# social-ai-uoft/sorrel

Hardware: AMD Instinct MI355X
Metric: agent-steps/sec (higher is better)
Workload: dtype u8 grid, f32 obs

## Files before the change

sorrel_amd/csrc/common.h:

```cpp
#pragma once


constexpr int kBlock = 256;
constexpr int kWave = 64;
constexpr int kMaxPass = 2;

struct DevTables {
    uint32_t thr_lo[SGW_MAX_TYPES];
    uint32_t delta[4][SGW_MAX_TYPES];
    double value[SGW_MAX_TYPES];
    uint8_t spawn_choice[SGW_MAX_TYPES][SGW_MAX_CHOICES];
    uint8_t spawn_count[SGW_MAX_TYPES];
    uint8_t agent_type[SGW_MAX_AGENTS];
    uint8_t dense_choice[SGW_MAX_CHOICES];
    uint8_t layer_fill[8];
    uint8_t layer_border[8];
    uint8_t pad_[8];
    uint8_t rule[SGW_MAX_TYPES];
    int8_t rule_layer[SGW_MAX_TYPES];
    uint8_t rule_become[SGW_MAX_TYPES];
    uint8_t pad2_[SGW_MAX_TYPES];
    uint32_t rule_mask[SGW_MAX_TYPES];
    uint32_t delta3[SGW_MAX_TYPES];
    double appearance[SGW_MAX_TYPES][SGW_MAX_CHANNELS];
// ... 13 lines not shown
    int64_t row[SGW_MAX_AGENTS];
    int64_t cap[SGW_MAX_AGENTS];
    int64_t step[SGW_MAX_AGENTS];
    void* states[SGW_MAX_AGENTS];
    float* rewards[SGW_MAX_AGENTS];
    int64_t* actions[SGW_MAX_AGENTS];
    float* dones[SGW_MAX_AGENTS];
    int64_t row_elems[SGW_MAX_AGENTS];
    uint64_t eps_thr[SGW_MAX_AGENTS];
};

struct RowPtrs {
    void* p[SGW_MAX_AGENTS];
    int64_t stride;
    const void* agent_action;
    int action_kind;
    float* reward_row;
    int64_t* action_row;
    const TurnState* ts;
    const TurnState* ets;
    int dual;
    int rows_mode2;
};

struct Params {
    int H, W, L, A, r, V, VV, C, T, nact, zA;
    int cells;
    int64_t env_stride;
    int cells_pad;
    int env_lds;
    int tab_bytes;
    uint32_t default_type, fill_type;
    uint32_t spawn_mask, thr_full_mask, pass_mask;
    uint32_t become_mask;
    uint32_t agent_mask;
    uint32_t dy_pack, dx_pack;
    uint32_t fill_delta[4];
    uint32_t fill_delta3;
    uint32_t fill_delta16[2];
    uint32_t spawn_pat;
    uint32_t spawn_thr;
    uint32_t spawn_full;
    uint32_t spawn_n;
    uint32_t choice_lo, choice_hi;
    uint32_t seed_lo, seed_hi;
    uint32_t first_env;
    int64_t E;
    uint32_t epoch, turn, flags;
    int a0, a1;
    int do_move;
    int obs_post;
    int obs_u8;
    int agent_rule;
    uint32_t tag_it, tag_notit;
    double tag_reward;
    uint8_t* agent_state;
    uint8_t* agent_dir;
    int has_become;
    uint32_t quiet0, quiet1;
    uint32_t kind_pack;
    int beam_radius;
    uint32_t clean_beam, zap_beam, beam_block_mask;
    int total_factor;
    uint8_t* state_at_pov;
    uint64_t dense_thr;
    int dense_count;
    uint8_t* grid;
    uint8_t* pos;
    uint8_t* actions;
    float* obs;
    float* rewards;
    double* total;
    const DevTables* tab;
    const uint8_t* tmpl;
    int* status;
    int obs_stage;
    int stage_agents;
    int obs_next;
    int obs_A, obs_a0;
    int64_t obs_ag;
    int big_pitch;
    int big_stage;
    int big_stage_off;
    uint32_t* walk_ctr;
    int walk_word;
    int walk_static;
    int single_spawner;
    int rows_mode;
    int rows_by_agent;
    int onehot;
    int tail_kind, tail_len;
    const float* tail_table;
    const TurnState* ts;
    uint32_t nturns;
    int64_t ts_obs, ts_act, ts_rew;
    uint32_t extras;
    uint32_t drawn_mask;
    uint8_t* target_types;
};
constexpr uint32_t kExtraDrawn = 1u, kExtraTargets = 2u;
#ifdef SGW_JIT
constexpr bool kExtrasDefault = false;
#else
constexpr bool kExtrasDefault = true;
#endif
constexpr bool extras_default_tables(const int tc) { return kExtrasDefault && tc == 0; }
template <bool XTRAS>
__device__ __forceinline__ uint32_t extras_of(const Params& p) {
    if constexpr (XTRAS) return p.extras;
    else return 0u;
}

struct U4 {
    uint32_t x, y, z, w;
};

__device__ __forceinline__ uint32_t xor3(uint32_t a, uint32_t b, uint32_t k) {
    uint32_t d;
    asm("v_bitop3_b32 %0, %1, %2, %3 bitop3:0x96" : "=v"(d) : "v"(a), "v"(b), "s"(k));
    return d;
}

template <bool OWN_KEYS = true>
__device__ __forceinline__ U4 philox4x32_10(uint32_t c0, uint32_t c1, uint32_t c2, uint32_t c3,
                                            uint32_t k0, uint32_t k1) {
#ifndef SGW_DIAG_SHARED_KEYS
    if constexpr (OWN_KEYS) asm volatile("" : "+s"(k0), "+s"(k1));
#endif
#pragma unroll
    for (int r = 0; r < 10; ++r) {
        const uint64_t p0 = (uint64_t)0xD2511F53u * c0;
        const uint64_t p1 = (uint64_t)0xCD9E8D57u * c2;
        const uint32_t n0 = xor3((uint32_t)(p1 >> 32), c1, k0);
        const uint32_t n2 = xor3((uint32_t)(p0 >> 32), c3, k1);
        c1 = (uint32_t)p1;
        c3 = (uint32_t)p0;
        c0 = n0;
        c2 = n2;
        k0 += 0x9E3779B9u;
        k1 += 0xBB67AE85u;
    }
    return U4{c0, c1, c2, c3};
}

__device__ __forceinline__ uint32_t opaque(uint32_t v) {
    asm volatile("" : "+v"(v));
    return v;
}

__device__ __forceinline__ uint32_t word_of(const U4& v, int i) {
    return i == 0 ? v.x : i == 1 ? v.y : i == 2 ? v.z : v.w;
}

__device__ __forceinline__ uint32_t value_draw(const Params& p, const uint32_t cell, const uint32_t turn, const uint32_t env_id, const uint32_t ep4) {
    const U4 w = philox4x32_10(cell >> 2, turn, env_id, ep4 | SGW_STREAM_VALUE, p.seed_lo, p.seed_hi);
    return word_of(w, (int)(cell & 3u));
}
__device__ __forceinline__ double drawn_value(const DevTables* gtab, const uint32_t t, const uint32_t u, const double otherwise) {
    return (uint64_t)u < gtab->alt_thr[t & 31u] ? gtab->value_alt[t & 31u] : otherwise;
}

__device__ __forceinline__ float obs_finish(double acc, int post) {
    if (post == SGW_OBS_POST_CLIP255_DIV255) acc = fmin(fmax(acc, 0.0), 255.0) / 255.0;
    return (float)acc;
}

template <int WPE>
__device__ __forceinline__ void gsync() {
    if constexpr (WPE == 1) {
        __builtin_amdgcn_fence(__ATOMIC_ACQ_REL, "wavefront");
        __builtin_amdgcn_wave_barrier();
    } else {
        __syncthreads();
    }
}

template <int G>
__device__ __forceinline__ void load_grid(const Params& p, const uint8_t* __restrict__ src,
                                          uint8_t* lds, int gtid) {
    if ((p.env_stride & 15) == 0 && p.env_stride >= p.cells_pad) {
        const uint4* s = reinterpret_cast<const uint4*>(src);
        uint4* d = reinterpret_cast<uint4*>(lds);
        const int nu = p.cells_pad >> 4;
        for (int i = gtid; i < nu; i += G) {
            uint4 v = s[i];
            if (i == nu - 1 && (p.cells & 15)) {
                const int tail = p.cells & 15;
                uint32_t w[4] = {v.x, v.y, v.z, v.w};
#pragma unroll
                for (int q = 0; q < 4; ++q) {
                    const int keep = tail - 4 * q;
                    if (keep <= 0) w[q] = 0xFFFFFFFFu;
                    else if (keep < 4) w[q] |= 0xFFFFFFFFu << (8 * keep);
                }
                v = make_uint4(w[0], w[1], w[2], w[3]);
            }
            d[i] = v;
        }
    } else if ((p.cells & 3) == 0 && (p.env_stride & 3) == 0) {
        const uint32_t* s = reinterpret_cast<const uint32_t*>(src);
        uint32_t* d = reinterpret_cast<uint32_t*>(lds);
        for (int i = gtid; i < (p.cells >> 2); i += G) d[i] = s[i];
    } else {
        for (int i = gtid; i < p.cells_pad; i += G) lds[i] = i < p.cells ? src[i] : (uint8_t)0xFF;
    }
}

template <int G>
__device__ __forceinline__ void store_grid(const Params& p, uint8_t* __restrict__ dst,
                                           const uint8_t* lds, int gtid) {
    if ((p.env_stride & 15) == 0 && p.env_stride >= p.cells_pad) {
        uint4* d = reinterpret_cast<uint4*>(dst);
        const uint4* s = reinterpret_cast<const uint4*>(lds);
        for (int i = gtid; i < (p.cells_pad >> 4); i += G) d[i] = s[i];
    } else if ((p.cells & 3) == 0 && (p.env_stride & 3) == 0) {
        uint32_t* d = reinterpret_cast<uint32_t*>(dst);
        const uint32_t* s = reinterpret_cast<const uint32_t*>(lds);
        for (int i = gtid; i < (p.cells >> 2); i += G) d[i] = s[i];
    } else {
        for (int i = gtid; i < p.cells; i += G) dst[i] = lds[i];
    }
}


template <int G>
__device__ __forceinline__ void sweep_single(const Params& p, uint8_t* lds_grid, uint32_t env_id, int gtid, uint32_t turn, const uint32_t ep4,
                                             uint32_t* through = nullptr,
                                             const int d0 = 0) {
    uint32_t* g32 = reinterpret_cast<uint32_t*>(lds_grid);
    const int ndw = (p.cells + 3) >> 2;
    for (int d = d0 + gtid; d < ndw; d += G) {
        const uint32_t dv = g32[d], pat = p.spawn_pat & 0xFFu;
        const bool m0 = (dv & 0xFFu) == pat, m1 = ((dv >> 8) & 0xFFu) == pat, m2 = ((dv >> 16) & 0xFFu) == pat, m3 = (dv >> 24) == pat;
        if (!(m0 | m1 | m2 | m3)) continue;
        const U4 w = philox4x32_10((uint32_t)d, turn, env_id, ep4 | SGW_STREAM_SPAWN, p.seed_lo, p.seed_hi);
        const bool f = p.spawn_full != 0;
        uint32_t hits = 0;
        hits |= (m0 && (f || w.x < p.spawn_thr)) ? 1u : 0u;
        hits |= (m1 && (f || w.y < p.spawn_thr)) ? 2u : 0u;
        hits |= (m2 && (f || w.z < p.spawn_thr)) ? 4u : 0u;
        hits |= (m3 && (f || w.w < p.spawn_thr)) ? 8u : 0u;
        if (hits == 0) continue;
        const U4 k = philox4x32_10((uint32_t)d, turn, env_id, ep4 | SGW_STREAM_SPAWN_KIND, p.seed_lo, p.seed_hi);
#pragma unroll
        for (int b = 0; b < 4; ++b)
            if ((hits >> b) & 1u) {
                const uint32_t pick = __umulhi(word_of(k, b), p.spawn_n);
                lds_grid[4 * d + b] = (uint8_t)(((pick < 4 ? p.choice_lo : p.choice_hi) >> (8 * (pick & 3u))) & 0xFFu);
            }
        if (through) through[d] = g32[d];
    }
}

template <int G>
__device__ __forceinline__ void sweep(const Params& p, const DevTables* tab, uint8_t* lds_grid,
                                      uint32_t env_id, int gtid, uint32_t turn, const uint32_t ep4) {
    uint32_t* g32 = reinterpret_cast<uint32_t*>(lds_grid);
    const int ndw = (p.cells + 3) >> 2;
    const uint32_t c3 = ep4 | SGW_STREAM_SPAWN;
    for (int d = gtid; d < ndw; d += G) {
        uint32_t v = g32[d];
        uint32_t m = 0;
#pragma unroll
        for (int b = 0; b < 4; ++b) {
            const uint32_t t = (v >> (8 * b)) & 0xFFu;
            const uint32_t is = (t < SGW_MAX_TYPES) ? ((p.spawn_mask >> t) & 1u) : 0u;
            m |= is << b;
        }
        if (m == 0) continue;
        const U4 w = philox4x32_10((uint32_t)d, turn, env_id, c3, p.seed_lo, p.seed_hi);
        uint32_t hits = 0;
#pragma unroll
        for (int b = 0; b < 4; ++b) {
            if ((m >> b) & 1u) {
                const uint32_t t = (v >> (8 * b)) & 31u;
                const bool hit = ((p.thr_full_mask >> t) & 1u) || (word_of(w, b) < tab->thr_lo[t]);
                hits |= (hit ? 1u : 0u) << b;
            }
        }
        if (hits == 0) continue;
        const U4 k = philox4x32_10((uint32_t)d, turn, env_id, ep4 | SGW_STREAM_SPAWN_KIND,
                                   p.seed_lo, p.seed_hi);
#pragma unroll
        for (int b = 0; b < 4; ++b) {
            if ((hits >> b) & 1u) {
                const uint32_t t = (v >> (8 * b)) & 31u;
                const uint32_t n = tab->spawn_count[t];
                const uint32_t pick = (uint32_t)(((uint64_t)word_of(k, b) * n) >> 32);
                const uint32_t nt = tab->spawn_choice[t][pick];
                v = (v & ~(0xFFu << (8 * b))) | (nt << (8 * b));
            }
        }
        g32[d] = v;
    }
}

template <int WPE, int G, typename Tab>
__device__ __forceinline__ void sweep_ordered(const Params& p, const Tab* rt, uint8_t* lg, const uint32_t env_id, const int gtid,
                                              const uint32_t turn, const uint32_t ep4, const int L, const int HW) {
    const uint32_t* lg32 = reinterpret_cast<const uint32_t*>(lg);
    for (int z = 0; z < L; ++z) {
        const int lo = z * HW, hi = lo + HW;
        for (int d = (lo >> 2) + gtid; d < ((hi + 3) >> 2); d += G) {
            const uint32_t word = lg32[d];
            if (word == p.quiet0 || word == p.quiet1) continue;
            uint32_t tj[4];
// ... 54 lines not shown
```

sorrel_amd/csrc/step_fast.h:

```cpp
#pragma once

constexpr int kMaxUnits = 4;
constexpr int kMaxUnitsRules = 8;
constexpr int kMaxUnitsPlain = 11;
constexpr size_t kLdsPerCu = 160 * 1024;
constexpr size_t kCacheResidentGrid = (size_t)288 << 20;

#define OBS_STORE(ptr, val) (*(ptr) = (val))


template <bool OWN_KEYS>
__device__ __forceinline__ uint32_t sweep_hits(const uint4& u, const uint32_t unit, const Params& p, const uint32_t env_id, const uint32_t turn, const uint32_t ep4) {
    uint32_t hits = 0;
    const uint32_t pat = p.spawn_pat & 0xFFu;
#pragma unroll
    for (int k = 0; k < 4; ++k) {
        const uint32_t dv = k == 0 ? u.x : k == 1 ? u.y : k == 2 ? u.z : u.w;
        const bool m0 = (dv & 0xFFu) == pat, m1 = ((dv >> 8) & 0xFFu) == pat, m2 = ((dv >> 16) & 0xFFu) == pat, m3 = (dv >> 24) == pat;
        if (m0 | m1 | m2 | m3) {
            const U4 w = philox4x32_10<OWN_KEYS>(opaque(unit * 4 + k), turn, env_id, ep4 | SGW_STREAM_SPAWN, p.seed_lo, p.seed_hi);
            const bool f = p.spawn_full != 0;
            uint32_t hb = 0;
            hb |= (m0 && (f || w.x < p.spawn_thr)) ? 1u : 0u;
            hb |= (m1 && (f || w.y < p.spawn_thr)) ? 2u : 0u;
            hb |= (m2 && (f || w.z < p.spawn_thr)) ? 4u : 0u;
            hb |= (m3 && (f || w.w < p.spawn_thr)) ? 8u : 0u;
            hits |= hb << (4 * k);
        }
    }
    return hits;
}

template <bool OWN_KEYS>
__device__ __forceinline__ void sweep_apply(uint32_t hits, const uint32_t unit, uint8_t* lg, const Params& p,
                                            const uint32_t env_id, const uint32_t turn, const uint32_t ep4) {
    while (hits) {
        const uint32_t cell = (uint32_t)__ffs(hits) - 1u;
        hits &= hits - 1u;
        const uint32_t off = unit * 16u + cell;
        const U4 kw = philox4x32_10<OWN_KEYS>(opaque(off >> 2), turn, env_id, ep4 | SGW_STREAM_SPAWN_KIND, p.seed_lo, p.seed_hi);
        const uint32_t pick = __umulhi(word_of(kw, off & 3u), p.spawn_n);
        lg[off] = (uint8_t)(((pick < 4 ? p.choice_lo : p.choice_hi) >> (8 * (pick & 3u))) & 0xFFu);
    }
}

#ifdef SGW_STAMPS
constexpr int kStampEnvs = 65536;
__device__ unsigned long long g_stamps[kStampEnvs * 8];
#define STAMP(i)                                                                                             \
    do {                                                                                                     \
        __builtin_amdgcn_sched_barrier(0);                                                                   \
        unsigned long long t_;                                                                               \
        asm volatile("s_memrealtime %0\n\ts_waitcnt lgkmcnt(0)" : "=s"(t_)::"memory");                             \
        __builtin_amdgcn_sched_barrier(0);                                                                   \
        if (lane == 0 && (i) > 0 && env < kStampEnvs) g_stamps[env * 8 + (i)-1] = t_ - tprev_;                \
        tprev_ = t_;                                                                                         \
    } while (0)
#else
#define STAMP(i)
#endif

#ifndef SGW_FAST_RULES_PLAIN_WAVES
#define SGW_FAST_RULES_PLAIN_WAVES 6
#endif
#ifndef SGW_FAST_MULTI_WAVES
#define SGW_FAST_MULTI_WAVES 6
#endif
template <int TL, int TC, int TR, int TH, int TW, bool TAIL = false>
__device__ __forceinline__ void fast_rows_emit(const Params& p, const RowPtrs* rp, uint8_t* smem, const int sub, const int lane) {
    typedef float vfloat4 __attribute__((ext_vector_type(4)));
    typedef float vfloat2 __attribute__((ext_vector_type(2)));
    constexpr int kN = TC * (2 * TR + 1) * (2 * TR + 1);
    const int ob_off = p.tab_bytes + ((TL * TH * TW + 15) & ~15);
    const int64_t env_first = (int64_t)blockIdx.x * 4;
    const int live = (int)(p.E - env_first < 4 ? p.E - env_first : 4);
    __syncthreads();
    auto emit_run = [&](float* dst, const int a, const int k0, const int n) {
        const uintptr_t ad = reinterpret_cast<uintptr_t>(dst);
        const int T = n * kN;
        auto src16 = [&](const int t) -> uint32_t {
            const int k = t / (kN / 2), j2 = t - k * (kN / 2);
            return *reinterpret_cast<const uint16_t*>(smem + (k0 + k) * p.env_lds + ob_off + a * kN + 2 * j2);
        };
        if ((kN & 1) == 0 && (ad & 15u) == 0) {
            const int q = T >> 2;
            const int mis = (int)((ad >> 4) & 7u);
            for (int i = lane - mis; i < q; i += 64) {
                if (i < 0) continue;
                const uint32_t lo = src16(2 * i), hi = src16(2 * i + 1);
                vfloat4 v;
                v.x = (float)(lo & 0xFFu);
                v.y = (float)(lo >> 8);
                v.z = (float)(hi & 0xFFu);
                v.w = (float)(hi >> 8);
                __builtin_nontemporal_store(v, reinterpret_cast<vfloat4*>(dst) + i);
            }
            if ((T & 3) && lane == 0) {
                const uint32_t b = src16(2 * q);
                vfloat2 v;
                v.x = (float)(b & 0xFFu);
                v.y = (float)(b >> 8);
                __builtin_nontemporal_store(v, reinterpret_cast<vfloat2*>(dst) + 2 * q);
            }
        } else if ((kN & 1) == 0 && (ad & 7u) == 0) {
            const int mis = (int)((ad >> 3) & 15u);
            for (int i = lane - mis; i < (T >> 1); i += 64) {
                if (i < 0) continue;
                const uint32_t b = src16(i);
                vfloat2 v;
                v.x = (float)(b & 0xFFu);
                v.y = (float)(b >> 8);
                __builtin_nontemporal_store(v, reinterpret_cast<vfloat2*>(dst) + i);
            }
        } else {
            for (int i = lane; i < T; i += 64) {
                const int k = i / kN, j = i - k * kN;
                __builtin_nontemporal_store((float)smem[(k0 + k) * p.env_lds + ob_off + a * kN + j], dst + i);
            }
        }
    };
    for (int a = sub; a < p.A; a += 4) {
        float* base = static_cast<float*>(rp->p[a]) + env_first * rp->stride;
        if (rp->stride == kN) emit_run(base, a, 0, live);
        else for (int k = 0; k < live; ++k) emit_run(base + k * rp->stride, a, k, 1);
        if (rp->dual && rp->ts->cap[a] > 0 && rp->ts->states[a]) {
            const int64_t re = rp->ts->row_elems[a];
            float* ring = static_cast<float*>(rp->ts->states[a]) + (rp->ts->row[a] * p.E + env_first) * re;
            if (re == kN) emit_run(ring, a, 0, live);
            else for (int k = 0; k < live; ++k) emit_run(ring + k * re, a, k, 1);
        }
        if constexpr (TAIL) if (p.tail_kind != SGW_TAIL_NONE && rp->stride >= kN + p.tail_len) {
            for (int k = 0; k < live; ++k) {
                float* t = base + k * rp->stride + kN;
                const int64_t ea = (env_first + k) * p.A + a;
                if (p.tail_kind == SGW_TAIL_AGENT_IS_IT) {
                    if (lane == 0) t[0] = (p.agent_state && p.agent_state[ea] == p.tag_it) ? 1.f : 0.f;
                } else {
                    const uint32_t yx = reinterpret_cast<const uint16_t*>(p.pos)[ea];
                    const float* src = p.tail_table + ((int64_t)(yx & 0xFFu) * TW + (yx >> 8)) * p.tail_len;
                    for (int j = lane; j < p.tail_len; j += 64) t[j] = src[j];
                }
            }
        }
    }
}

template <bool ONEHOT, int TL, int TC, int TR, int TH, int TW, bool TAG, bool RULES, bool STAGE, bool MULTI, bool P3, bool I16, bool ROWS, bool ROWX = false, bool TAIL = false, bool XTRAS = kExtrasDefault>
__device__ __forceinline__ void step_fast_body(const Params p, [[maybe_unused]] const RowPtrs* rp) {
    static_assert(!ROWS || (ONEHOT && TL && TC && TH && TW && !RULES && !STAGE && !MULTI && !P3 && !I16), "ROWS: plain or Tag movers, one-hot, compile-time shape");
    static_assert(!ROWX || (ONEHOT && STAGE && !MULTI && !I16 && !ROWS), "ROWX: a chunk-staging single-turn instance");
    extern __shared__ __attribute__((aligned(16))) uint8_t smem[];
    const int tid = threadIdx.x;
    const int lane = tid & 63;
    const int sub = __builtin_amdgcn_readfirstlane(tid >> 6);
    const int64_t env = (int64_t)blockIdx.x * 4 + sub;
    if (env >= p.E) {
        if constexpr (ROWS)
            if (p.obs_stage > 0 && p.a0 == 0 && p.a1 == p.A && !(p.flags & SGW_STEP_NO_OBS))
                fast_rows_emit<TL, TC, TR, TH, TW, TAIL>(p, rp, smem, sub, lane);
        return;
    }
#ifdef SGW_STAMPS
    unsigned long long tprev_ = 0;
    STAMP(0);
    if (lane == 0 && env < kStampEnvs) {
        g_stamps[env * 8 + 6] = tprev_;
        g_stamps[env * 8 + 7] = (unsigned long long)__builtin_amdgcn_s_getreg(63492) | ((unsigned long long)__builtin_amdgcn_s_getreg(63508) << 32);
    }
#endif

    const int L = TL ? TL : p.L;
    const int C = TC ? TC : p.C;
    const int r = TR ? TR : p.r;
    const int V = 2 * r + 1, VV = V * V;
    const int H = TH ? TH : p.H, W = TW ? TW : p.W, HW = H * W;
    constexpr bool kStatic = TL && TH && TW;
    constexpr bool kOwnKeys = !kStatic;
    const int cells = kStatic ? TL * TH * TW : p.cells;
    const int nunits = (cells + 15) >> 4;
    constexpr int NU = kStatic ? ((TL * TH * TW + 15) / 16 + 63) / 64 : kMaxUnits;
    constexpr int kFullRounds = kStatic ? ((TL * TH * TW + 15) / 16) / 64 : 0;
    constexpr int kTailUnits = kStatic ? ((TL * TH * TW + 15) / 16) % 64 : 0;
    constexpr bool kTailDword = kStatic && !RULES && kTailUnits > 0 && kTailUnits <= 48;
    const int zoff = p.zA * HW;
    static_assert(!I16 || (ONEHOT && !P3 && !RULES && !(TL && TH && TW)), "I16: a byte-staging instance with run-time map");
    constexpr int NW = P3 ? 1 : I16 ? 2 : (TC ? (TC + 3) / 4 : 4);
    constexpr int CMAX = P3 ? (TC ? TC : 10) : I16 ? (TC ? TC : 4) : 4 * NW;

    uint8_t* wl = smem + sub * p.env_lds;
    const DevTables* gtab = p.tab;
    const uint32_t env_id = p.first_env + (uint32_t)env;
    uint32_t turn0 = p.turn, ep4 = p.epoch << 4;
    if (p.ts) { turn0 = p.ts->turn + 1u; ep4 = p.ts->epoch << 4; }

    uint4 u[NU];
    {
        const uint4* src = reinterpret_cast<const uint4*>(p.grid + env * p.env_stride);
#pragma unroll
        for (int k = 0; k < NU; ++k)
            if (lane + 64 * k < nunits) u[k] = src[lane + 64 * k];
    }
    const bool mine = lane >= p.a0 && lane < p.a1 && lane < p.A;
    const bool rnd = (p.flags & SGW_STEP_RANDOM_ACTIONS) != 0;
    uint32_t yx = 0, act = 0;
    if (lane < p.A) yx = reinterpret_cast<const uint16_t*>(p.pos)[env * p.A + lane];
    if ((yx & 0xFFu) >= (uint32_t)H || (yx >> 8) >= (uint32_t)W) {
        yx = 0;
        atomicOr(p.status, SGW_STATUS_BAD_POS);
    }
    if (mine && p.do_move && !rnd) act = p.actions[env * p.A + lane];
    const double vtab = gtab->value[lane & 31];
    uint32_t atype = gtab->agent_type[lane];
    if (p.agent_state && lane < p.A) atype = p.agent_state[env * p.A + lane];
    uint32_t pov_type = atype;
    if constexpr (ONEHOT) {
        uint32_t* wd = reinterpret_cast<uint32_t*>(wl);
        if constexpr (I16) {
            wd[lane] = reinterpret_cast<const uint32_t*>(gtab->delta16)[lane];
            float* l = reinterpret_cast<float*>(smem + 4 * p.env_lds);
#pragma unroll
            for (int j = 0; j < 4; ++j) l[lane + 64 * j] = gtab->post_lut[lane + 64 * j];
        } else if constexpr (P3) {
            if (lane < SGW_MAX_TYPES) wd[lane] = gtab->delta3[lane];
        } else {
#pragma unroll
            for (int q = 0; q < (NW + 1) / 2; ++q) wd[lane + 64 * q] = reinterpret_cast<const uint32_t*>(gtab->delta)[lane + 64 * q];
        }
    } else {
        double* wa = reinterpret_cast<double*>(wl);
        for (int i = lane; i < SGW_MAX_TYPES * SGW_MAX_CHANNELS; i += 64) wa[i] = reinterpret_cast<const double*>(gtab->appearance)[i];
    }
    const uint32_t* wdelta = reinterpret_cast<const uint32_t*>(wl);
    [[maybe_unused]] const float* post_lut = reinterpret_cast<const float*>(smem + 4 * p.env_lds);
    auto tof = [&](const uint32_t k) -> float {
        if constexpr (I16) return post_lut[k];
        else return (float)k;
    };
    const double(*wapp)[SGW_MAX_CHANNELS] = reinterpret_cast<const double(*)[SGW_MAX_CHANNELS]>(wl);
    uint8_t* lg = wl + p.tab_bytes + (RULES ? kRuleLds : 0);
    uint4* lg16 = reinterpret_cast<uint4*>(lg);
    [[maybe_unused]] const RuleLds* rt = reinterpret_cast<const RuleLds*>(wl + p.tab_bytes);
    [[maybe_unused]] uint32_t adir = 2;
    [[maybe_unused]] uint32_t kind_v = 0;
    if constexpr (RULES) {
        uint32_t* rd = reinterpret_cast<uint32_t*>(wl + p.tab_bytes);
        const uint32_t* gA = reinterpret_cast<const uint32_t*>(gtab->thr_lo);
        const uint32_t* gB = reinterpret_cast<const uint32_t*>(gtab->spawn_choice);
        const uint32_t* gC = reinterpret_cast<const uint32_t*>(gtab->rule);
        if (lane < 32) rd[lane] = gA[lane];
        rd[32 + lane] = gB[lane];
        if (lane < 8) rd[96 + lane] = gB[64 + lane];
        rd[104 + lane] = gC[lane];
        if (p.agent_dir && lane < p.A) adir = p.agent_dir[env * p.A + lane];
    }
    uint8_t* ob = lg + ((cells + 15) & ~15);
    constexpr bool kStageAlways = ONEHOT && STAGE;
    const bool stage = kStageAlways || (ONEHOT && kStatic && p.obs_stage > 0 && p.a0 == 0 && p.a1 == p.A);
#ifdef SGW_DIAG_NO_LINE_ALIGN
    constexpr uint32_t kLineMask = 3u;
#else
    constexpr uint32_t kLineMask = 31u;
#endif
    [[maybe_unused]] int ch_a0 = 0;
    [[maybe_unused]] uint32_t ch_shift = 0;
    [[maybe_unused]] uint32_t ch_lo = 0;
    if constexpr (kStageAlways) ch_lo = ch_shift = (uint32_t)(env * (int64_t)(p.A * C * VV)) & kLineMask;
    [[maybe_unused]] float* row_dst = nullptr;

    int wdi[2], wdj[2], woff[2];
#pragma unroll
    for (int k = 0; k < 2; ++k) {
        const int w = lane + 64 * k;
        const int i = w / V, j = w - i * V;
        wdi[k] = i - r;
        wdj[k] = j - r;
        woff[k] = wdi[k] * W + wdj[k];
    }
    const uint32_t vt_lo = (uint32_t)__double_as_longlong(vtab), vt_hi = (uint32_t)(__double_as_longlong(vtab) >> 32);
    const uint32_t vt_f32 = __float_as_uint((float)vtab);
    const bool write_obs = !(p.flags & SGW_STEP_NO_OBS);
    const bool do_sweep = (p.flags & SGW_STEP_SWEEP) != 0;
    const bool dirty = do_sweep || (p.do_move && p.a1 > p.a0);
    const bool sweep_only = !RULES && (MULTI ? p.nturns : 1u) == 1u && !(p.do_move && p.a1 > p.a0);

    {
        double tot = p.do_move ? p.total[env] : 0.0;

#ifdef SGW_STAMPS
        asm volatile("s_waitcnt vmcnt(0)" ::: "memory");
#endif
        STAMP(1);
        [[maybe_unused]] uint32_t hits[NU];
        if constexpr (!kStatic || ((TL * TH * TW) & 15) != 0) {
            if (cells & 15) {
#pragma unroll
                for (int k = 0; k < NU; ++k)
                    if (lane + 64 * k == nunits - 1) {
                        const int tail = cells & 15;
                        uint32_t d[4] = {u[k].x, u[k].y, u[k].z, u[k].w};
#pragma unroll
                        for (int q = 0; q < 4; ++q) {
                            const int keep = tail - 4 * q;
                            if (keep <= 0) d[q] = 0xFFFFFFFFu;
                            else if (keep < 4) d[q] |= 0xFFFFFFFFu << (8 * keep);
                        }
                        u[k] = make_uint4(d[0], d[1], d[2], d[3]);
                    }
            }
        }
#pragma unroll
        for (int k = 0; k < NU; ++k)
            if (lane + 64 * k < nunits) lg16[lane + 64 * k] = u[k];
        if constexpr (RULES || !kStatic) {
            const uint4* src = reinterpret_cast<const uint4*>(p.grid + env * p.env_stride);
            for (int i = 64 * NU + lane; i < nunits; i += 64) {
                uint4 v = src[i];
                if ((cells & 15) && i == nunits - 1) {
                    const int tail = cells & 15;
                    uint32_t d[4] = {v.x, v.y, v.z, v.w};
#pragma unroll
                    for (int q = 0; q < 4; ++q) {
                        const int keep = tail - 4 * q;
                        if (keep <= 0) d[q] = 0xFFFFFFFFu;
                        else if (keep < 4) d[q] |= 0xFFFFFFFFu << (8 * keep);
                    }
                    v = make_uint4(d[0], d[1], d[2], d[3]);
                }
                lg16[i] = v;
            }
        }
        int st_lane = 0;
        uint32_t taddr_v = 0xFFFFFFFFu, oaddr_v = 0, npos = 0, rew_bits = 0, moved = 0;
        const uint32_t nturns = MULTI ? p.nturns : 1u;
        for (uint32_t tix = 0; tix < nturns; ++tix) {
        const uint32_t turn = turn0 + tix;
        if constexpr (RULES) {
            gsync<1>();
            if (do_sweep) {
                sweep_ordered<1, 64>(p, rt, lg, env_id, lane, turn, ep4, L, HW);
            }
        } else if constexpr (!kStatic) {
            gsync<1>();
            if (do_sweep) {
                sweep_single<64>(p, lg, env_id, lane, turn, ep4,
                                 sweep_only ? reinterpret_cast<uint32_t*>(p.grid + env * p.env_stride) : nullptr);
                gsync<1>();
            }
        } else {
            if (tix > 0) {
                gsync<1>();
#pragma unroll
                for (int k = 0; k < NU; ++k)
                    if (lane + 64 * k < nunits) u[k] = lg16[lane + 64 * k];
            }
#pragma unroll
            for (int k = 0; k < NU; ++k) {
                hits[k] = 0;
                if ((k < kFullRounds || !kTailDword) && lane + 64 * k < nunits && do_sweep)
                    hits[k] = sweep_hits<kOwnKeys>(u[k], (uint32_t)(lane + 64 * k), p, env_id, turn, ep4);
            }
            gsync<1>();
            if (do_sweep) {
                auto kind_draw = [&](const uint32_t b) {
                    const uint32_t off = ((uint32_t)lane + 64u * (b >> 4)) * 16u + (b & 15u);
                    const U4 kw = philox4x32_10<kOwnKeys>(opaque(off >> 2), turn, env_id, ep4 | SGW_STREAM_SPAWN_KIND, p.seed_lo, p.seed_hi);
                    const uint32_t pick = __umulhi(word_of(kw, off & 3u), p.spawn_n);
                    lg[off] = (uint8_t)(((pick < 4 ? p.choice_lo : p.choice_hi) >> (8 * (pick & 3u))) & 0xFFu);
                };
                if constexpr (NU <= 2) {
                    uint32_t hm = hits[0];
                    if constexpr (NU == 2) hm |= hits[1] << 16;
                    while (hm) {
                        const uint32_t b = (uint32_t)__ffs(hm) - 1u;
                        hm &= hm - 1u;
                        kind_draw(b);
                    }
                } else {
                    static_assert(NU <= 4, "16 hit bits per unit, four units per lane");
                    uint64_t hm = 0;
#pragma unroll
                    for (int k = 0; k < NU; ++k) hm |= (uint64_t)hits[k] << (16 * k);
                    while (hm) {
                        const uint32_t b = (uint32_t)__ffsll((unsigned long long)hm) - 1u;
                        hm &= hm - 1ull;
                        kind_draw(b);
                    }
                }
                if constexpr (kTailDword)
                    sweep_single<64>(p, lg, env_id, lane, turn, ep4, sweep_only ? reinterpret_cast<uint32_t*>(p.grid + env * p.env_stride) : nullptr,
                                     256 * kFullRounds);
                gsync<1>();
            }
        }

        STAMP(2);
        const uint32_t py = yx & 0xFFu, px = yx >> 8;
        taddr_v = 0xFFFFFFFFu;
        npos = yx;
        if (p.do_move && mine) {
            if (rnd) {
                const U4 w = philox4x32_10<kOwnKeys>(opaque((uint32_t)lane >> 2), turn, env_id, ep4 | SGW_STREAM_ACTION,
                                           p.seed_lo, p.seed_hi);
                act = __umulhi(word_of(w, lane & 3), (uint32_t)p.nact);
                p.actions[tix * p.ts_act + env * p.A + lane] = (uint8_t)act;
            } else if (tix > 0) {
                act = p.actions[tix * p.ts_act + env * p.A + lane];
            }
            const bool act_ok = act < (uint32_t)p.nact;
            int dy = (int)((p.dy_pack >> (2 * (act & 15u))) & 3u) - 1;
            int dx = (int)((p.dx_pack >> (2 * (act & 15u))) & 3u) - 1;
            if constexpr (RULES) {
                if (p.agent_rule == SGW_AGENT_RULE_CLEANUP) {
                    const uint32_t kind = act_ok ? (p.kind_pack >> (2 * (act & 15u))) & 3u : 0u;
                    if (kind != SGW_ACTION_MOVE || !act_ok) dy = dx = 0;
                    const uint32_t ndir = (dy == -1 && dx == 0) ? 0u : (dy == 1 && dx == 0) ? 2u : (dy == 0 && dx == -1) ? 3u : (dy == 0 && dx == 1) ? 1u : 4u;
                    kind_v = kind | (act_ok ? 4u : 0u) | (ndir << 4);
                }
            }
            const int ty = (int)py + dy, tx = (int)px + dx;
            const bool inb = (unsigned)ty < (unsigned)H && (unsigned)tx < (unsigned)W;
            if (act_ok && inb) {
                taddr_v = (uint32_t)(zoff + ty * W + tx);
                npos = (uint32_t)ty | ((uint32_t)tx << 8);
            }
            st_lane |= !act_ok ? SGW_STATUS_BAD_ACTION : (!inb ? SGW_STATUS_OOB_MOVE : 0);
        }
        oaddr_v = (uint32_t)zoff + py * (uint32_t)W + px;
        uint32_t xv = 255u;
        if (extras_of<XTRAS>(p) & kExtraDrawn) {
            if (taddr_v != 0xFFFFFFFFu) xv = value_draw(p, taddr_v, turn, env_id, ep4);
        }
        rew_bits = 0;
        moved = 0;
        const int64_t turn_obs = tix * p.ts_obs;
        if constexpr (kStageAlways) {
            ch_a0 = 0;
            ch_lo = ch_shift = (uint32_t)(turn_obs + env * (int64_t)(p.A * C * VV)) & kLineMask;
        }

        STAMP(3);
        [[maybe_unused]] auto emit_chunk = [&](const int a_lo, const int a_hi, const bool last) {
            gsync<1>();
            typedef float vfloat4 __attribute__((ext_vector_type(4)));
            const int N = (a_hi - a_lo) * C * VV;
            const int64_t e0 = turn_obs + (env * p.A + a_lo) * (int64_t)(C * VV);
            const int sh = (int)ch_shift, lo = (int)ch_lo;
            const int hi = sh + N;
            const int he = last ? hi : (hi & ~(int)kLineMask);
            if (he <= lo) {
                ch_shift = (uint32_t)hi;
                return;
            }
            const uint32_t* ob4 = reinterpret_cast<const uint32_t*>(ob);
            const int i0 = (lo + 3) >> 2, i1 = he >> 2;
            const int ie = lane == 0 ? i0 - 1 : i1;
            const bool edge = lane == 0 ? (lo & 3) != 0 : (lane == 1 && (he & 3) != 0 && (i1 >= i0 || (lo & 3) == 0));
            if (ROWX || !p.obs_u8) {
                float* gb = ROWX ? row_dst - sh : p.obs + (e0 - sh);
                for (int i = lane; i < i1; i += 64) {
                    if (i < i0) continue;
                    const uint32_t b = ob4[i];
                    vfloat4 v;
                    v.x = tof(b & 0xFFu);
                    v.y = tof((b >> 8) & 0xFFu);
                    v.z = tof((b >> 16) & 0xFFu);
                    v.w = tof(b >> 24);
#ifdef SGW_DIAG_PLAIN_STORES
                    *reinterpret_cast<vfloat4*>(gb + 4 * i) = v;
#else
                    __builtin_nontemporal_store(v, reinterpret_cast<vfloat4*>(gb + 4 * i));
#endif
                }
                if (edge) {
                    const uint32_t b = ob4[ie];
#pragma unroll
                    for (int j = 0; j < 4; ++j)
                        if (4 * ie + j >= lo && 4 * ie + j < he) gb[4 * ie + j] = tof((b >> (8 * j)) & 0xFFu);
                }
            } else {
                uint8_t* gb = reinterpret_cast<uint8_t*>(p.obs) + (e0 - sh);
                for (int i = lane; i < i1; i += 64) {
                    if (i < i0) continue;
                    __builtin_nontemporal_store(ob4[i], reinterpret_cast<uint32_t*>(gb + 4 * i));
                }
                if (edge) {
                    const uint32_t b = ob4[ie];
#pragma unroll
                    for (int j = 0; j < 4; ++j)
                        if (4 * ie + j >= lo && 4 * ie + j < he) gb[4 * ie + j] = (uint8_t)(b >> (8 * j));
                }
            }
            if constexpr (ROWX) {
                if (p.tail_kind != SGW_TAIL_NONE) {
                    float* t = row_dst + C * VV;
                    if (p.tail_kind == SGW_TAIL_AGENT_IS_IT) {
                        const uint32_t ty_ = (uint32_t)__builtin_amdgcn_readlane((int)atype, a_lo);
                        if (lane == 0) t[0] = ty_ == p.tag_it ? 1.f : 0.f;
                    } else {
                        const int ay_ = __builtin_amdgcn_readlane((int)(yx & 0xFFu), a_lo), ax_ = __builtin_amdgcn_readlane((int)(yx >> 8), a_lo);
                        const float* src = p.tail_table + ((int64_t)ay_ * W + ax_) * p.tail_len;
                        for (int k = lane; k < p.tail_len; k += 64) t[k] = src[k];
                    }
                }
            }
            if (!last) {
                uint8_t t = 0;
                if (lane < hi - he) t = ob[he + lane];
                gsync<1>();
                if (lane < hi - he) ob[lane] = t;
                ch_shift = (uint32_t)(hi - he);
                ch_lo = 0;
            }
            gsync<1>();
        };
        const int a_end = (p.obs_next && p.a1 < p.A) ? p.a1 + 1 : p.a1;
        for (int a = p.a0; a < a_end; ++a) {
            if constexpr (ROWX) {
                if (a > p.a0 && write_obs) emit_chunk(a - 1, a, true);
                ch_a0 = a;
                row_dst = static_cast<float*>(rp->p[a]) + env * rp->stride;
                ch_lo = ch_shift = (uint32_t)(reinterpret_cast<uintptr_t>(row_dst) >> 2) & kLineMask;
            } else if constexpr (kStageAlways) {
                if (a - ch_a0 == p.stage_agents) {
                    if (write_obs) emit_chunk(ch_a0, a, false);
                    ch_a0 = a;
                }
            }
            const int s_o = __builtin_amdgcn_readlane((int)oaddr_v, a);
            if (p.obs_next ? a == p.a1 : write_obs) {
                const int y = __builtin_amdgcn_readlane((int)py, a);
                const int x = __builtin_amdgcn_readlane((int)px, a);
                const int cbase = s_o - zoff;
                float* obase = p.obs + turn_obs + ((env * p.obs_A + (a - p.obs_a0)) * (int64_t)C) * VV;
#pragma unroll
                for (int k = 0; k < 2; ++k) {
                    if (64 * k >= VV) break;
                    const int w = lane + 64 * k;
                    if (w < VV) {
#ifdef SGW_DIAG_SKIP_GATHER
                        if (p.turn != 0xFFFFFFFFu) continue;
#endif
                        const bool inb = (unsigned)(y + wdi[k]) < (unsigned)H && (unsigned)(x + wdj[k]) < (unsigned)W;
                        const int off = inb ? cbase + woff[k] : 0;
                        float* o = obase + w;
                        if constexpr (ONEHOT) {
                            uint32_t cnt[NW];
#pragma unroll
                            for (int q = 0; q < NW; ++q) cnt[q] = 0;
#pragma unroll
                            for (int z = 0; z < (TL ? TL : 1); ++z) {
                                const uint32_t t = lg[z * HW + off] & 31u;
#pragma unroll
                                for (int q = 0; q < NW; ++q) cnt[q] += wdelta[q * 32 + t];
                            }
                            if constexpr (TL == 0) {
                                for (int z = 1; z < L; ++z) {
                                    const uint32_t t = lg[z * HW + off] & 31u;
#pragma unroll
                                    for (int q = 0; q < NW; ++q) cnt[q] += wdelta[q * 32 + t];
                                }
                            }
#pragma unroll
                            for (int q = 0; q < NW; ++q) cnt[q] = inb ? cnt[q] : (P3 ? p.fill_delta3 : I16 ? p.fill_delta16[q] : p.fill_delta[q]);
                            auto chan = [&](const int c) -> uint32_t {
                                if constexpr (P3) return (cnt[0] >> (3 * c)) & 7u;
                                else if constexpr (I16) return min((cnt[c >> 1] >> (16 * (c & 1))) & 0xFFFFu, 255u);
                                else return (cnt[c >> 2] >> (8 * (c & 3))) & 0xFFu;
                            };
                            if (stage) {
                                uint8_t* os = ob + (kStageAlways ? (int)ch_shift + ((a - ch_a0) * C) * VV : (a * C) * VV) + w;
                                if constexpr (TC != 0) {
#pragma unroll
                                    for (int c = 0; c < CMAX; ++c)
                                        if (c < C) os[c * VV] = (uint8_t)chan(c);
                                } else {
#pragma unroll
                                    for (int g = 0; g < (CMAX + 3) / 4; ++g)
                                        if (4 * g < C) {
#pragma unroll
                                            for (int b = 0; b < 4; ++b)
                                                if (4 * g + b < CMAX) os[(4 * g + b) * VV] = (uint8_t)chan(4 * g + b);
                                        }
                                }
                            } else if constexpr (kStageAlways) {
                            } else if (!p.obs_u8) {
#pragma unroll
                                for (int c = 0; c < CMAX; ++c)
                                    if (c < C) OBS_STORE(o + c * VV, tof(chan(c)));
                            } else {
                                uint8_t* o8 = reinterpret_cast<uint8_t*>(p.obs) + (o - p.obs);
#pragma unroll
                                for (int c = 0; c < CMAX; ++c)
                                    if (c < C) o8[c * VV] = (uint8_t)chan(c);
                            }
                        } else {
                            for (int c = 0; c < C; ++c) {
                                double acc = wapp[lg[off] & 31u][c];
                                for (int z = 1; z < L; ++z) acc += wapp[lg[z * HW + off] & 31u][c];
                                OBS_STORE(o + c * VV, obs_finish(inb ? acc : wapp[p.fill_type][c], p.obs_post));
                            }
                        }
                    }
                }
            }
            if (!p.do_move || a >= p.a1) continue;
            const uint32_t s_t = (uint32_t)__builtin_amdgcn_readlane((int)taddr_v, a);
            const uint32_t my_type = (uint32_t)__builtin_amdgcn_readlane((int)atype, a);
            const bool valid = s_t != 0xFFFFFFFFu;
            if constexpr (RULES) {
                if (p.agent_rule == SGW_AGENT_RULE_CLEANUP) {
                    const uint32_t kd = (uint32_t)__builtin_amdgcn_readlane((int)kind_v, a);
                    const uint32_t kind = kd & 3u, ndir = kd >> 4;
                    const bool aok = (kd & 4u) != 0;
                    const uint32_t facing = (uint32_t)__builtin_amdgcn_readlane((int)adir, a) & 3u;
                    const int ay = __builtin_amdgcn_readlane((int)py, a), ax = __builtin_amdgcn_readlane((int)px, a);
                    if (aok && kind != SGW_ACTION_MOVE && p.zA + 1 < L) {
                        if (lane < 3 * p.beam_radius) {
                            const int arm = lane / p.beam_radius, i = lane - arm * p.beam_radius;
                            const int fy = facing == 0 ? -1 : facing == 2 ? 1 : 0, fx = facing == 1 ? 1 : facing == 3 ? -1 : 0;
                            const int ry = facing == 1 ? 1 : facing == 3 ? -1 : 0, rx = facing == 0 ? 1 : facing == 2 ? -1 : 0;
                            const int step = arm == 0 ? i + 1 : i, side = arm == 0 ? 0 : (arm == 1 ? 1 : -1);
                            const int by = ay + side * ry + step * fy, bx = ax + side * rx + step * fx;
                            if ((unsigned)by < (unsigned)H && (unsigned)bx < (unsigned)W) {
                                const int boff = (p.zA + 1) * HW + by * W + bx;
                                if (!((p.beam_block_mask >> (lg[boff] & 31u)) & 1u))
                                    lg[boff] = (uint8_t)(kind == SGW_ACTION_CLEAN ? p.clean_beam : p.zap_beam);
                            }
                        }
                        gsync<1>();
                    }
                    double val = 0.0;
                    uint32_t t = 0xFFu;
                    if (valid) {
                        const int tc = (int)s_t - zoff;
                        for (int zl = 0; zl < L; ++zl) {
                            const uint32_t tz = (uint32_t)__builtin_amdgcn_readfirstlane((int)lg[zl * HW + tc]) & 31u;
                            const uint32_t lo_ = (uint32_t)__builtin_amdgcn_readlane((int)vt_lo, (int)tz);
                            const uint32_t hi_ = (uint32_t)__builtin_amdgcn_readlane((int)vt_hi, (int)tz);
                            val += __longlong_as_double(((long long)hi_ << 32) | lo_);
                        }
                        t = (uint32_t)__builtin_amdgcn_readfirstlane((int)lg[s_t]);
                    }
                    const bool pass = valid && t < (uint32_t)p.T && ((p.pass_mask >> (t & 31u)) & 1u);
                    if (pass && lane == 0) {
                        lg[s_t] = (uint8_t)my_type;
                        lg[s_o] = (uint8_t)p.default_type;
                    }
                    moved = lane == a ? (pass ? 1u : 0u) : moved;
                    adir = (lane == a && aok && kind == SGW_ACTION_MOVE && ndir < 4u) ? ndir : adir;
                    rew_bits = lane == a ? __float_as_uint((float)val) : rew_bits;
                    tot += val * (double)(p.total_factor - 1);
                    tot += val;
                    gsync<1>();
                    continue;
                }
            }
            const uint32_t t = (uint32_t)__builtin_amdgcn_readfirstlane((int)lg[valid ? s_t : (uint32_t)s_o]);
            const bool tok = valid && t < (uint32_t)p.T;
            const uint32_t tl = t & 31u;
            uint32_t v_lo = (uint32_t)__builtin_amdgcn_readlane((int)vt_lo, (int)tl);
            uint32_t v_hi = (uint32_t)__builtin_amdgcn_readlane((int)vt_hi, (int)tl);
            uint32_t v_f = (uint32_t)__builtin_amdgcn_readlane((int)vt_f32, (int)tl);
            if constexpr (!TAG) {
                if (extras_of<XTRAS>(p)) {
                    if (tok && ((p.drawn_mask >> tl) & 1u)) {
                        const uint32_t u = (uint32_t)__builtin_amdgcn_readlane((int)xv, a);
                        const double dv = drawn_value(gtab, tl, u, __longlong_as_double(((long long)v_hi << 32) | v_lo));
                        v_lo = (uint32_t)__double_as_longlong(dv);
                        v_hi = (uint32_t)(__double_as_longlong(dv) >> 32);
                        v_f = __float_as_uint((float)dv);
                    }
                    xv = lane == a ? (valid ? t : 255u) : xv;
                }
            }
            const bool pass = tok && ((p.pass_mask >> tl) & 1u);
            if (pass && lane == 0) {
                lg[s_t] = (uint8_t)my_type;
                lg[s_o] = (uint8_t)p.default_type;
            }
            moved = lane == a ? (pass ? 1u : 0u) : moved;
            if constexpr (!TAG) {
                if (tok) tot += __longlong_as_double(((long long)v_hi << 32) | v_lo);
                rew_bits = lane == a ? (tok ? v_f : 0u) : rew_bits;
            } else {
                gsync<1>();
                pov_type = lane == a ? my_type : pov_type;
                const uint32_t np_a = (uint32_t)__builtin_amdgcn_readlane((int)npos, a);
                const int cy = pass ? (int)(np_a & 0xFFu) : (int)(((uint32_t)s_o - (uint32_t)zoff) / (uint32_t)W);
                const int cx = pass ? (int)((np_a >> 8) & 0xFFu) : (int)(((uint32_t)s_o - (uint32_t)zoff) % (uint32_t)W);
                const int own = zoff + cy * W + cx;
                int dstar = -1;
                if (my_type == p.tag_it) {
                    uint32_t nt[4];
                    bool ain[4];
#pragma unroll
                    for (int d = 0; d < 4; ++d) {
                        const int ay = cy + (d == 0 ? -1 : d == 2 ? 1 : 0), ax = cx + (d == 1 ? 1 : d == 3 ? -1 : 0);
                        ain[d] = (unsigned)ay < (unsigned)H && (unsigned)ax < (unsigned)W;
                        nt[d] = (uint32_t)__builtin_amdgcn_readfirstlane((int)lg[ain[d] ? zoff + ay * W + ax : own]);
                    }
#pragma unroll
                    for (int d = 3; d >= 0; --d)
                        if (ain[d] && nt[d] == p.tag_notit) dstar = d;
                }
                uint32_t mine_now = my_type;
                if (my_type == p.tag_it && dstar >= 0) {
                    const int ay = cy + (dstar == 0 ? -1 : dstar == 2 ? 1 : 0), ax = cx + (dstar == 1 ? 1 : dstar == 3 ? -1 : 0);
                    if (lane == 0) {
                        lg[own] = (uint8_t)p.tag_notit;
                        lg[zoff + ay * W + ax] = (uint8_t)p.tag_it;
                    }
                    const uint32_t curpos = moved ? npos : yx;
                    const uint32_t key = (uint32_t)ay | ((uint32_t)ax << 8);
                    atype = (lane < p.A && lane != a && curpos == key) ? p.tag_it : atype;
                    atype = lane == a ? p.tag_notit : atype;
                    mine_now = p.tag_notit;
                }
                const double val = mine_now != p.tag_it ? p.tag_reward : 0.0;
                tot += val;
                rew_bits = lane == a ? __float_as_uint((float)val) : rew_bits;
            }
            if (valid && !tok) st_lane |= SGW_STATUS_BAD_TYPE;
            gsync<1>();
        }

        STAMP(4);
        if constexpr (kStageAlways) {
            if (write_obs) emit_chunk(ch_a0, p.a1, true);
        } else if (stage && write_obs) {
            gsync<1>();
            const int nd = (p.A * C * VV) >> 2;
            const uint32_t* ob4 = reinterpret_cast<const uint32_t*>(ob);
            if constexpr (ROWS) {
                fast_rows_emit<TL, TC, TR, TH, TW, TAIL>(p, rp, smem, sub, lane);
            } else if (!p.obs_u8) {
                typedef float vfloat4 __attribute__((ext_vector_type(4)));
                vfloat4* o4 = reinterpret_cast<vfloat4*>(p.obs + turn_obs + env * (int64_t)(p.A * C * VV));
                const int mis = (int)((reinterpret_cast<uintptr_t>(o4) >> 4) & 7u);
                for (int i = lane - mis; i < nd; i += 64) {
                    if (i < 0) continue;
                    const uint32_t b = ob4[i];
                    vfloat4 v;
                    v.x = (float)(b & 0xFFu);
                    v.y = (float)((b >> 8) & 0xFFu);
                    v.z = (float)((b >> 16) & 0xFFu);
                    v.w = (float)(b >> 24);
                    __builtin_nontemporal_store(v, &o4[i]);
                }
            } else {
                uint32_t* o1 = reinterpret_cast<uint32_t*>(reinterpret_cast<uint8_t*>(p.obs) + turn_obs + env * (int64_t)(p.A * C * VV));
                for (int i = lane; i < nd; i += 64) __builtin_nontemporal_store(ob4[i], &o1[i]);
            }
        }
        if (p.do_move && mine) {
            p.rewards[tix * p.ts_rew + env * p.A + lane] = __uint_as_float(rew_bits);
            if constexpr (!TAG)
                if (extras_of<XTRAS>(p) & kExtraTargets) p.target_types[env * p.A + lane] = (uint8_t)xv;
            if (p.state_at_pov) p.state_at_pov[env * p.A + lane] = (uint8_t)pov_type;
        }
        if (tix + 1 < nturns) yx = moved ? npos : yx;
        }
        if (dirty) {
            if (!TAG && !RULES && !do_sweep && nturns == 1) {
                if (mine && moved) {
                    uint8_t* g = p.grid + env * p.env_stride;
                    g[oaddr_v] = lg[oaddr_v];
                    g[taddr_v] = lg[taddr_v];
                }
            } else if (sweep_only) {
                if constexpr (kStatic) {
                    uint4* dst = reinterpret_cast<uint4*>(p.grid + env * p.env_stride);
#pragma unroll
                    for (int k = 0; k < NU; ++k)
                        if (lane + 64 * k < nunits && hits[k]) dst[lane + 64 * k] = lg16[lane + 64 * k];
                }
            } else {
                uint4* dst = reinterpret_cast<uint4*>(p.grid + env * p.env_stride);
#pragma unroll
                for (int k = 0; k < NU; ++k)
                    if (lane + 64 * k < nunits) dst[lane + 64 * k] = lg16[lane + 64 * k];
                if constexpr (RULES || !kStatic)
                    for (int i = 64 * NU + lane; i < nunits; i += 64) dst[i] = lg16[i];
            }
        }
        if (p.do_move) {
            if (mine) {
                reinterpret_cast<uint16_t*>(p.pos)[env * p.A + lane] = (uint16_t)(moved ? npos : yx);
                if (st_lane) atomicOr(p.status, st_lane);
            }
            if (TAG && p.agent_state && lane < p.A) p.agent_state[env * p.A + lane] = (uint8_t)atype;
            if (RULES && p.agent_dir && lane < p.A) p.agent_dir[env * p.A + lane] = (uint8_t)adir;
            if (lane == 0) p.total[env] = tot;
        }
        STAMP(5);
#ifdef SGW_STAMPS
        asm volatile("s_waitcnt vmcnt(0)" ::: "memory");
#endif
        STAMP(6);
    }
}

template <bool ONEHOT, int TL, int TC, int TR, int TH, int TW, bool TAG = false, bool RULES = false, bool STAGE = false, bool MULTI = false, bool P3 = false, bool I16 = false>
__global__ __launch_bounds__(kBlock, MULTI ? SGW_FAST_MULTI_WAVES : (RULES ? (STAGE ? 7 : SGW_FAST_RULES_PLAIN_WAVES) : 8)) void step_fast(const Params p) {
    step_fast_body<ONEHOT, TL, TC, TR, TH, TW, TAG, RULES, STAGE, MULTI, P3, I16, false, false, false, extras_default_tables(TC)>(p, nullptr);
}
#ifdef SGW_JIT
template <bool ONEHOT, int TL, int TC, int TR, int TH, int TW, bool TAG = false, bool RULES = false, bool STAGE = false, bool MULTI = false, bool P3 = false, bool I16 = false>
__global__ __launch_bounds__(kBlock, MULTI ? SGW_FAST_MULTI_WAVES : (RULES ? (STAGE ? 7 : SGW_FAST_RULES_PLAIN_WAVES) : 8)) void step_fast_x(const Params p) {
    step_fast_body<ONEHOT, TL, TC, TR, TH, TW, TAG, RULES, STAGE, MULTI, P3, I16, false, false, false, true>(p, nullptr);
}
#endif

template <int TL, int TC, int TR, int TH, int TW, bool TAG, bool RULES, bool P3>
__global__ __launch_bounds__(kBlock, RULES ? 7 : 8) void step_fast_rowsx(const Params p, const RowPtrs rp) {
    step_fast_body<true, TL, TC, TR, TH, TW, TAG, RULES, true, false, P3, false, false, true, false, false>(p, &rp);
}

template <int TL, int TC, int TR, int TH, int TW, bool TAG = false, bool TAIL = false>
__global__ __launch_bounds__(kBlock, 8) void step_fast_rows(const Params p, const RowPtrs rp) {
    step_fast_body<true, TL, TC, TR, TH, TW, TAG, false, false, false, false, false, true, false, TAIL, false>(p, &rp);
}
```

Measured before the change: 4.479 billion.

## Fuse spawn-kind and action draws, scalarize per-agent bookkeeping, skip clean grid writeback

Packs the spawn hit offsets into a compact list in LDS, then draws spawn kinds and agent actions together in one wave-wide philox pass instead of a serial per-lane hit loop plus a separate action draw. Per-agent moved, reward and status bookkeeping now uses v_writelane through m0, and the agent position is taken from yx instead of separate readlanes. The fill deltas are hoisted into registers, and writeback of 1 KB grid units is skipped when they hold no agents and no spawn hits. The fused path adds a ballot-driven compaction loop and extra branching, and the inline asm writelane needs scalar operands.

```diff
diff --git a/sorrel_amd/csrc/common.h b/sorrel_amd/csrc/common.h
--- a/sorrel_amd/csrc/common.h
+++ b/sorrel_amd/csrc/common.h
@@ -189,6 +189,14 @@
     return i == 0 ? v.x : i == 1 ? v.y : i == 2 ? v.z : v.w;
 }
 
+__device__ __forceinline__ uint32_t write_lane(uint32_t v, const uint32_t val, const int lane) {
+    asm("s_mov_b32 m0, %2\n\ts_nop 0\n\tv_writelane_b32 %0, %1, m0"
+        : "+v"(v)
+        : "s"(__builtin_amdgcn_readfirstlane((int)val)), "s"(__builtin_amdgcn_readfirstlane(lane))
+        : "m0");
+    return v;
+}
+
 __device__ __forceinline__ uint32_t value_draw(const Params& p, const uint32_t cell, const uint32_t turn, const uint32_t env_id, const uint32_t ep4) {
     const U4 w = philox4x32_10(cell >> 2, turn, env_id, ep4 | SGW_STREAM_VALUE, p.seed_lo, p.seed_hi);
     return word_of(w, (int)(cell & 3u));
diff --git a/sorrel_amd/csrc/step_fast.h b/sorrel_amd/csrc/step_fast.h
--- a/sorrel_amd/csrc/step_fast.h
+++ b/sorrel_amd/csrc/step_fast.h
@@ -145,6 +145,11 @@
     }
 }
 
+template <bool WIDE> struct HitMask { typedef uint32_t type; };
+template <> struct HitMask<true> { typedef uint64_t type; };
+__device__ __forceinline__ uint32_t hm_first(const uint32_t m) { return (uint32_t)__ffs(m) - 1u; }
+__device__ __forceinline__ uint32_t hm_first(const uint64_t m) { return (uint32_t)__ffsll((unsigned long long)m) - 1u; }
+
 template <bool ONEHOT, int TL, int TC, int TR, int TH, int TW, bool TAG, bool RULES, bool STAGE, bool MULTI, bool P3, bool I16, bool ROWS, bool ROWX = false, bool TAIL = false, bool XTRAS = kExtrasDefault>
 __device__ __forceinline__ void step_fast_body(const Params p, [[maybe_unused]] const RowPtrs* rp) {
     static_assert(!ROWS || (ONEHOT && TL && TC && TH && TW && !RULES && !STAGE && !MULTI && !P3 && !I16), "ROWS: plain or Tag movers, one-hot, compile-time shape");
@@ -334,6 +339,8 @@
         const uint32_t nturns = MULTI ? p.nturns : 1u;
         for (uint32_t tix = 0; tix < nturns; ++tix) {
         const uint32_t turn = turn0 + tix;
+        constexpr uint32_t kNotDrawn = 0xFFFFFFFFu;
+        if (rnd) act = kNotDrawn;
         if constexpr (RULES) {
             gsync<1>();
             if (do_sweep) {
@@ -361,29 +368,57 @@
             }
             gsync<1>();
             if (do_sweep) {
-                auto kind_draw = [&](const uint32_t b) {
-                    const uint32_t off = ((uint32_t)lane + 64u * (b >> 4)) * 16u + (b & 15u);
-                    const U4 kw = philox4x32_10<kOwnKeys>(opaque(off >> 2), turn, env_id, ep4 | SGW_STREAM_SPAWN_KIND, p.seed_lo, p.seed_hi);
-                    const uint32_t pick = __umulhi(word_of(kw, off & 3u), p.spawn_n);
-                    lg[off] = (uint8_t)(((pick < 4 ? p.choice_lo : p.choice_hi) >> (8 * (pick & 3u))) & 0xFFu);
-                };
-                if constexpr (NU <= 2) {
-                    uint32_t hm = hits[0];
-                    if constexpr (NU == 2) hm |= hits[1] << 16;
+                typedef typename HitMask<(NU > 2)>::type hm_t;
+                static_assert(NU <= 4, "16 hit bits per unit, four units per lane");
+                hm_t hm = 0;
+#pragma unroll
+                for (int k = 0; k < NU; ++k) hm |= (hm_t)hits[k] << (16 * k);
+                auto unit_off = [&](const uint32_t b) { return ((uint32_t)lane + 64u * (b >> 4)) * 16u + (b & 15u); };
+                auto kind_of = [&](const uint32_t pick) { return (uint8_t)(((pick < 4 ? p.choice_lo : p.choice_hi) >> (8 * (pick & 3u))) & 0xFFu); };
+                uint32_t nlist = 0;
+                bool fused = false;
+                if constexpr (!ROWS && !MULTI) {
+                    uint32_t fl = p.flags;
+                    asm("" : "+s"(fl));
+                    if (stage && !(fl & SGW_STEP_NO_OBS) && p.do_move && rnd && p.a0 == 0 && p.a1 == p.A && p.obs_stage >= 256) {
+                        uint16_t* list = reinterpret_cast<uint16_t*>(ob);
+                        const uint32_t room = 64u - (uint32_t)p.A;
+                        hm_t rest = hm;
+                        uint64_t m = __ballot(rest != 0);
+                        while (m != 0 && nlist <= room) {
+                            if (rest != 0) {
+                                const uint32_t slot = nlist + __builtin_amdgcn_mbcnt_hi((uint32_t)(m >> 32), __builtin_amdgcn_mbcnt_lo((uint32_t)m, 0u));
+                                list[slot] = (uint16_t)unit_off(hm_first(rest));
+                                rest &= rest - 1u;
+                            }
+                            nlist += (uint32_t)__popcll(m);
+                            m = __ballot(rest != 0);
+                        }
+                        fused = m == 0 && nlist <= room;
+                    }
+                }
+                if (fused) {
+                    gsync<1>();
+                    const uint32_t na = (uint32_t)p.A;
+                    if ((uint32_t)lane < na + nlist) {
+                        const bool hit = (uint32_t)lane >= na;
+                        const uint32_t off = reinterpret_cast<const uint16_t*>(ob)[((uint32_t)lane - na) & 63u];
+                        const uint32_t ix = hit ? off : (uint32_t)lane;
+                        const U4 w = philox4x32_10<kOwnKeys>(opaque(ix >> 2), turn, env_id, ep4 | (hit ? SGW_STREAM_SPAWN_KIND : SGW_STREAM_ACTION), p.seed_lo, p.seed_hi);
+                        const uint32_t d = __umulhi(word_of(w, ix & 3u), hit ? p.spawn_n : (uint32_t)p.nact);
+                        if (hit) {
+                            lg[off] = kind_of(d);
+                        } else {
+                            act = d;
+                            p.actions[tix * p.ts_act + env * p.A + lane] = (uint8_t)d;
+                        }
+                    }
+                } else {
                     while (hm) {
-                        const uint32_t b = (uint32_t)__ffs(hm) - 1u;
+                        const uint32_t off = unit_off(hm_first(hm));
                         hm &= hm - 1u;
-                        kind_draw(b);
-                    }
-                } else {
-                    static_assert(NU <= 4, "16 hit bits per unit, four units per lane");
-                    uint64_t hm = 0;
-#pragma unroll
-                    for (int k = 0; k < NU; ++k) hm |= (uint64_t)hits[k] << (16 * k);
-                    while (hm) {
-                        const uint32_t b = (uint32_t)__ffsll((unsigned long long)hm) - 1u;
-                        hm &= hm - 1ull;
-                        kind_draw(b);
+                        const U4 kw = philox4x32_10<kOwnKeys>(opaque(off >> 2), turn, env_id, ep4 | SGW_STREAM_SPAWN_KIND, p.seed_lo, p.seed_hi);
+                        lg[off] = kind_of(__umulhi(word_of(kw, off & 3u), p.spawn_n));
                     }
                 }
                 if constexpr (kTailDword)
@@ -399,10 +434,12 @@
         npos = yx;
         if (p.do_move && mine) {
             if (rnd) {
-                const U4 w = philox4x32_10<kOwnKeys>(opaque((uint32_t)lane >> 2), turn, env_id, ep4 | SGW_STREAM_ACTION,
-                                           p.seed_lo, p.seed_hi);
-                act = __umulhi(word_of(w, lane & 3), (uint32_t)p.nact);
-                p.actions[tix * p.ts_act + env * p.A + lane] = (uint8_t)act;
+                if (act == kNotDrawn) {
+                    const U4 w = philox4x32_10<kOwnKeys>(opaque((uint32_t)lane >> 2), turn, env_id, ep4 | SGW_STREAM_ACTION,
+                                               p.seed_lo, p.seed_hi);
+                    act = __umulhi(word_of(w, lane & 3), (uint32_t)p.nact);
+                    p.actions[tix * p.ts_act + env * p.A + lane] = (uint8_t)act;
+                }
             } else if (tix > 0) {
                 act = p.actions[tix * p.ts_act + env * p.A + lane];
             }
@@ -432,6 +469,8 @@
         }
         rew_bits = 0;
         moved = 0;
+        constexpr bool kScalarBook = !TAG && !RULES;
+        [[maybe_unused]] uint32_t book = 0;
         const int64_t turn_obs = tix * p.ts_obs;
         if constexpr (kStageAlways) {
             ch_a0 = 0;
@@ -513,6 +552,12 @@
             }
             gsync<1>();
         };
+        [[maybe_unused]] uint32_t fill_v[NW];
+        constexpr bool kFillRegs = ONEHOT && kStatic && !RULES && !STAGE && !P3 && !I16;
+        if constexpr (kFillRegs) {
+#pragma unroll
+            for (int q = 0; q < NW; ++q) fill_v[q] = opaque(p.fill_delta[q]);
+        }
         const int a_end = (p.obs_next && p.a1 < p.A) ? p.a1 + 1 : p.a1;
         for (int a = p.a0; a < a_end; ++a) {
             if constexpr (ROWX) {
@@ -526,10 +571,10 @@
                     ch_a0 = a;
                 }
             }
-            const int s_o = __builtin_amdgcn_readlane((int)oaddr_v, a);
+            const uint32_t yx_a = (uint32_t)__builtin_amdgcn_readlane((int)yx, a);
+            const int y = (int)(yx_a & 0xFFu), x = (int)(yx_a >> 8);
+            const int s_o = zoff + y * W + x;
             if (p.obs_next ? a == p.a1 : write_obs) {
-                const int y = __builtin_amdgcn_readlane((int)py, a);
-                const int x = __builtin_amdgcn_readlane((int)px, a);
                 const int cbase = s_o - zoff;
                 float* obase = p.obs + turn_obs + ((env * p.obs_A + (a - p.obs_a0)) * (int64_t)C) * VV;
 #pragma unroll
@@ -561,7 +606,7 @@
                                 }
                             }
 #pragma unroll
-                            for (int q = 0; q < NW; ++q) cnt[q] = inb ? cnt[q] : (P3 ? p.fill_delta3 : I16 ? p.fill_delta16[q] : p.fill_delta[q]);
+                            for (int q = 0; q < NW; ++q) cnt[q] = inb ? cnt[q] : (kFillRegs ? fill_v[q] : P3 ? p.fill_delta3 : I16 ? p.fill_delta16[q] : p.fill_delta[q]);
                             auto chan = [&](const int c) -> uint32_t {
                                 if constexpr (P3) return (cnt[0] >> (3 * c)) & 7u;
                                 else if constexpr (I16) return min((cnt[c >> 1] >> (16 * (c & 1))) & 0xFFFFu, 255u);
@@ -670,7 +715,7 @@
                         v_hi = (uint32_t)(__double_as_longlong(dv) >> 32);
                         v_f = __float_as_uint((float)dv);
                     }
-                    xv = lane == a ? (valid ? t : 255u) : xv;
+                    xv = write_lane(xv, valid ? t : 255u, a);
                 }
             }
             const bool pass = tok && ((p.pass_mask >> tl) & 1u);
@@ -678,10 +723,12 @@
                 lg[s_t] = (uint8_t)my_type;
                 lg[s_o] = (uint8_t)p.default_type;
             }
-            moved = lane == a ? (pass ? 1u : 0u) : moved;
+            if constexpr (kScalarBook) book = write_lane(book, tok ? (p.pass_mask >> tl) & 1u : (valid ? 2u : 0u), a);
+            else moved = lane == a ? (pass ? 1u : 0u) : moved;
             if constexpr (!TAG) {
-                if (tok) tot += __longlong_as_double(((long long)v_hi << 32) | v_lo);
-                rew_bits = lane == a ? (tok ? v_f : 0u) : rew_bits;
+                tot += __longlong_as_double(tok ? (long long)(((uint64_t)v_hi << 32) | v_lo) : (long long)0x8000000000000000ull);
+                if constexpr (kScalarBook) rew_bits = write_lane(rew_bits, tok ? v_f : 0u, a);
+                else rew_bits = lane == a ? (tok ? v_f : 0u) : rew_bits;
             } else {
                 gsync<1>();
                 pov_type = lane == a ? my_type : pov_type;
@@ -720,8 +767,13 @@
                 tot += val;
                 rew_bits = lane == a ? __float_as_uint((float)val) : rew_bits;
             }
-            if (valid && !tok) st_lane |= SGW_STATUS_BAD_TYPE;
+            if constexpr (!kScalarBook)
+                if (valid && !tok) st_lane |= SGW_STATUS_BAD_TYPE;
             gsync<1>();
+        }
+        if constexpr (kScalarBook) {
+            moved = book & 1u;
+            if (book & 2u) st_lane |= SGW_STATUS_BAD_TYPE;
         }
 
         STAMP(4);
@@ -777,8 +829,15 @@
             } else {
                 uint4* dst = reinterpret_cast<uint4*>(p.grid + env * p.env_stride);
 #pragma unroll
-                for (int k = 0; k < NU; ++k)
+                for (int k = 0; k < NU; ++k) {
+                    if constexpr (kStatic && !RULES && !TAG && !MULTI) {
+                        if (k < kFullRounds && (k + 1) * 1024 <= TL * TH * TW) {
+                            const bool agents_here = zoff < (k + 1) * 1024 && zoff + HW > k * 1024;
+                            if (!agents_here && __ballot(hits[k] != 0) == 0) continue;
+                        }
+                    }
                     if (lane + 64 * k < nunits) dst[lane + 64 * k] = lg16[lane + 64 * k];
+                }
                 if constexpr (RULES || !kStatic)
                     for (int i = 64 * NU + lane; i < nunits; i += 64) dst[i] = lg16[i];
             }
```

New measurement: 4.618 billion, median of 6. 3.1% higher.
